# gouldberg/robotics-path-planning

Measured on AMD Instinct MI355X. Metric: RRT* edge expansions/sec + final path cost, 100k-node tree (collision-checked edges evaluated on the device, distinct per iteration; 105000 iterations), higher is better.
Workload: dtype f64

## Files before the change

### robotics-path-planning_amd/csrc/rrt_kernels.hip.h

```cpp
#pragma once
#include <hip/hip_runtime.h>
#include <stdint.h>

#include "rpp_core.h"
#include "rpp_node.h"
#include "rpp_rs.h"

namespace rppk {

constexpr int TPB = 256;
constexpr int NW = TPB / 64;
constexpr int UNROLL = 4;
constexpr int WAVE_STRIDE = 128 * UNROLL;
constexpr int MAX_OBS = 256;
constexpr int NU_MAX = 512;
constexpr int EB = 64;
constexpr int EBD = 32;
constexpr int FCAP = TPB;
constexpr double FILTER_EPS = 7.105427357601002e-15;

struct Result {
  double path_cost;
  int32_t n_nodes;
  int32_t status;
// ... 33 lines not shown
  int32_t *parent, *prev_sib;
  Kid* kid;
  GHead* ghead;
  int32_t *hits, *stack;
  int64_t stride;
  const double *ox, *oy, *othr;
  const double* r2tab;
  double* path_xy;
  int32_t path_cap;
  Result* results;
  int32_t algo, sampler, goal_sample_rate, max_iter, has_play, until_max;
  double rand_min, rand_max, expand_dis, res;
  double play_area[4];
  int32_t trace_inst;
  double *tr_rx, *tr_ry;
  int32_t *tr_near, *tr_nn;
  int32_t* tr_kind;
  float *xf, *yf;
  double f32_m;
  uint32_t* xq;
  double q_lo, q_inv, q_step, q_m;
  const int32_t* inst_map;
  int32_t spec2;
  uint64_t *gent, *gpool;
  int32_t gsh, gn, gcells, gpool_blocks;
  int32_t grid;
  int32_t grid_min;
  int32_t prop_vec, prop_cap;
  int32_t obs_cull;
  int32_t grid_merge;
  int32_t has_elen;
  Node* node;
  double* samp;
};
constexpr int GRID_CAP0 = 16, GRID_CAP1 = 16;

__device__ __forceinline__ uint32_t quant16(const Ctx& c, double px, double py) {
  double qx = __builtin_rint((px - c.q_lo) * c.q_inv), qy = __builtin_rint((py - c.q_lo) * c.q_inv);
  qx = qx < 0.0 ? 0.0 : (qx > 65535.0 ? 65535.0 : qx);
  qy = qy < 0.0 ? 0.0 : (qy > 65535.0 ? 65535.0 : qy);
  return ((uint32_t)qx | ((uint32_t)qy << 16)) ^ 0x80008000u;
}

struct Sh {
  static constexpr int kNU = NU_MAX, kTPB = TPB, kNW = NW;
  rpp::MT rng;
  double ox[MAX_OBS], oy[MAX_OBS], othr[MAX_OBS];
  rpp::Edge edge[EB];
  int32_t ecoll[EB];
  double uval[NU_MAX];
  int32_t uidx[NU_MAX];
  double uex[NU_MAX], uey[NU_MAX], uaux[NU_MAX];
  int32_t usafe[NU_MAX];
  double cval[TPB];
  int32_t cflag[TPB];
  double red_best[NW], red_second[NW];
  int32_t red_idx[NW];
  int32_t wave_cnt[NW];
  int32_t wave_start[NW];
  double rx, ry, nx, ny, ncost, wx, wy, wcost;
  int32_t ni, flag, nu, nvalid, sel, overflow;
  int32_t fa, fb, fover, fcount;
};

__device__ __forceinline__ int roundup_i(int a, int b) { return (a + b - 1) / b * b; }

typedef double v2d __attribute__((ext_vector_type(2)));
__device__ __forceinline__ v2d stream2(const double* p) {
// ... 1239 lines not shown
```

### robotics-path-planning_amd/csrc/rrt_star_v2_grid.inc

```
struct GridS {
  GHead* head;
  uint64_t* ent;
  uint64_t* pool;
  int sh, gn, pool_blocks, pool_next, excl, min_n;
  uint32_t goal_q;
  int ok;
  int merge;
  int bytes, nodes;
};
constexpr int GRID_CAP0 = rppk::GRID_CAP0, GRID_CAP1 = rppk::GRID_CAP1, GRID_CAPT = GRID_CAP0 + GRID_CAP1;
constexpr int GE = 4;
static_assert(GRID_CAPT <= 64, "a cell's entries fit one wave");

__device__ __forceinline__ GHead ld_head(const GHead* p) { return *p; }
__device__ __forceinline__ int grid_cell(const GridS& g, uint32_t q) {
  const uint32_t u = q ^ 0x80008000u;
  return (int)((u >> (16 + g.sh)) * (uint32_t)g.gn + ((u & 0xffffu) >> g.sh));
}
__device__ __forceinline__ uint64_t grid_entry(int node, uint32_t q) { return (uint64_t)(uint32_t)node | ((uint64_t)q << 32); }

__device__ __forceinline__ void grid_build(GridS& g, const uint32_t* __restrict__ xq, const double* x, const double* y,
                                           int n, double gx, double gy, int first_goal) {
  const int lane = threadIdx.x & 63;
  const int cells = g.gn * g.gn;
  for (int i = lane; i < cells; i += 64) {
    g.head[i] = GHead{0, 0};
  }
  g.pool_next = 0;
  g.excl = 0;
  __threadfence();
  const uint64_t lt_mask = (lane == 0) ? 0ull : (~0ull >> (64 - lane));
  for (int i0 = 0; i0 < n; i0 += 64) {
    const int i = i0 + lane;
    bool on = i < n;
    const uint32_t q = on ? xq[i] : 0u;
    if (on && first_goal >= 0 && q == g.goal_q && i != first_goal && x[i] == gx && y[i] == gy) on = false;
    g.excl += __popcll(__ballot(i < n && !on));
    const int cell = grid_cell(g, q);
    const int k = on ? atomicAdd(&g.head[cell].cnt, 1) : 0;
    const uint64_t nb = __ballot(on && k == GRID_CAP0);
    if (on && k == GRID_CAP0) {
// ... 28 lines not shown
        return;
      }
      b = ++g.pool_next;
    }
    if (threadIdx.x == 0) g.pool[(int64_t)(b - 1) * GRID_CAP1 + (k - GRID_CAP0)] = e;
  }
  if (threadIdx.x == 0) g.head[cell] = GHead{k + 1, b};
}

__device__ __forceinline__ void grid_remove(GridS& g, int node, uint32_t q) {
  const int lane = threadIdx.x & 63;
  const int cell = grid_cell(g, q);
  const GHead hd = ld_head(g.head + cell);
  const int k = hd.cnt, b = hd.blk;
  if (k > GRID_CAPT) {
    g.ok = 0;
    return;
  }
  uint64_t* p = lane < GRID_CAP0 ? g.ent + (int64_t)cell * GRID_CAP0 + lane
                                 : (b > 0 ? g.pool + (int64_t)(b - 1) * GRID_CAP1 + (lane - GRID_CAP0) : nullptr);
  const bool mine = lane < k && p != nullptr;
  const uint64_t e = mine ? *p : 0ull;
  const uint64_t m = __ballot(mine && (int)(uint32_t)e == node);
  if (m == 0ull) {
    g.ok = 0;
    return;
  }
  const int j = __ffsll((long long)m) - 1;
  const uint32_t lo = (uint32_t)__shfl((int)(uint32_t)e, k - 1), hi = (uint32_t)__shfl((int)(uint32_t)(e >> 32), k - 1);
  if (lane == j) *p = (uint64_t)lo | ((uint64_t)hi << 32);
  if (lane == 0) g.head[cell].cnt = k - 1;
}

__device__ __forceinline__ int grid_tests(const GridS& g, uint32_t cq, int D, bool ball, uint32_t thr, bool nearest,
                                          const uint32_t (&ev)[GE], const int (&ei)[GE], const uint32_t (&d)[GE],
                                          int32_t* __restrict__ hits, int off, int cap, int32_t* lhit, int32_t* ltmp,
                                          int gz, int& cnt, int& zcnt, uint32_t& best, uint32_t& second, int& grp,
                                          uint32_t& wbest) {
  const int lane = threadIdx.x & 63;
  const uint64_t lt_mask = (lane == 0) ? 0ull : (~0ull >> (64 - lane));
  if (ball) {
    const bool zin = g.excl > 0 && qdist(g.goal_q, cq) <= thr;
    if (zin && gz < 0) return 0;
    int z = zin ? g.excl : 0, H = 0;
    bool hh[GE];
#pragma unroll
    for (int k = 0; k < GE; k++) {
      hh[k] = d[k] <= thr;
      if (gz >= 0) {
        const bool skip = hh[k] && ev[k] == g.goal_q && ei[k] != gz;
        z += __popcll(__ballot(skip));
        hh[k] = hh[k] && !skip;
      }
      const uint64_t m = __ballot(hh[k]);
      if (hh[k]) ltmp[H + __popcll(m & lt_mask)] = ei[k];
      H += __popcll(m);
    }
    lds_barrier();
    for (int h0 = 0; h0 < H; h0 += 64) {
      if (h0 + lane < H) {
        const int me = ltmp[h0 + lane];
        int r = 0;
        for (int j = 0; j < H; j++) r += ltmp[j] < me ? 1 : 0;
        if (r < cap) hits[off + r] = me;
        if (lhit && r < HWF) lhit[r] = me;
      }
    }
    lds_barrier();
    cnt = H;
    zcnt = z;
  }
  if (!nearest) return 1;
  uint32_t b = 0xffffffffu, s = 0xffffffffu;
  int bi = 0x7fffffff;
#pragma unroll
  for (int k = 0; k < GE; k++) {
    if (d[k] < b || (d[k] == b && ei[k] < bi)) {
      s = b;
      b = d[k];
      bi = ei[k];
    } else {
      s = min(s, d[k]);
    }
  }
  uint32_t wb = b;
  int wi = bi;
#pragma unroll
  for (int o = 32; o >= 1; o >>= 1) {
    const uint32_t ob = (uint32_t)__shfl_xor((int)wb, o);
    const int oi = __shfl_xor(wi, o);
    const bool take = ob < wb || (ob == wb && oi < wi);
    wb = take ? ob : wb;
    wi = take ? oi : wi;
  }
  uint32_t ws = bi == wi ? s : b;
#pragma unroll
  for (int o = 32; o >= 1; o >>= 1) ws = min(ws, (uint32_t)__shfl_xor((int)ws, o));
  if (g.excl > 0) ws = min(ws, qdist(g.goal_q, cq));
  wbest = wb;
  if (wb < QSAT && (double)D > __builtin_sqrt((double)wb) + 4.0) {
    best = wb;
    second = min(ws, (uint32_t)(D * D));
    grp = wi & ~3;
    return 1;
  }
  return 2;
}

__device__ __forceinline__ bool grid_window(const GridS& g, uint32_t cq, int rw, int& x0, int& y0, int& nwx, int& nc, int& D) {
  const int ux = (int)((cq ^ 0x80008000u) & 0xffffu), uy = (int)((cq ^ 0x80008000u) >> 16);
  x0 = max(ux - rw, 0) >> g.sh;
  y0 = max(uy - rw, 0) >> g.sh;
  const int x1 = min(ux + rw, 65535) >> g.sh, y1 = min(uy + rw, 65535) >> g.sh;
  nwx = x1 - x0 + 1;
  nc = nwx * (y1 - y0 + 1);
  if (nc > 64) return false;
  D = 32767;
  if (x0 > 0) D = min(D, ux - (x0 << g.sh) + 1);
  if (x1 < g.gn - 1) D = min(D, ((x1 + 1) << g.sh) - ux);
  if (y0 > 0) D = min(D, uy - (y0 << g.sh) + 1);
  if (y1 < g.gn - 1) D = min(D, ((y1 + 1) << g.sh) - uy);
  return true;
}

__device__ __forceinline__ int grid_grow(uint32_t wb, int rw) { return wb < QSAT ? (int)__builtin_sqrt((double)wb) + 6 : 3 * rw + 1; }

__device__ __forceinline__ bool grid_centre(const GridS& g, uint32_t cq, int rw, bool ball, uint32_t thr, bool nearest,
                                            int32_t* __restrict__ hits, int off, int cap, int32_t* lhit, int32_t* ltmp,
                                            int gz, int& cnt, int& zcnt, uint32_t& best, uint32_t& second, int& grp,
                                            int& bytes, int& nodes, int first_attempt = 0) {
  const int lane = threadIdx.x & 63;
  for (int attempt = first_attempt; attempt < 3; attempt++) {
    int x0, y0, nwx, nc, D;
    if (!grid_window(g, cq, rw, x0, y0, nwx, nc, D)) return false;
    int cell = 0, cn = 0, cb = 0;
    if (lane < nc) {
      cell = (y0 + lane / nwx) * g.gn + x0 + lane % nwx;
      const GHead hd = ld_head(g.head + cell);
      cn = hd.cnt;
      cb = hd.blk;
    }
    if (__ballot(cn > GRID_CAPT) != 0ull) return false;
    int inc = cn;
#pragma unroll
    for (int o = 1; o < 64; o <<= 1) {
      const int t = __shfl_up(inc, o);
      if (lane >= o) inc += t;
    }
    const int tot = __shfl(inc, 63);
    bytes += 8 * nc + 8 * tot;
    nodes += tot;
    if (tot > 64 * GE) return false;
    const int pre = inc - cn;
    const uint64_t* ptr[GE];
#pragma unroll
    for (int k = 0; k < GE; k++) ptr[k] = nullptr;
    for (uint64_t nz = __ballot(cn > 0); nz != 0ull; nz &= nz - 1) {
      const int j = __ffsll((long long)nz) - 1;
      const int pj = __builtin_amdgcn_readlane(pre, j), cj = __builtin_amdgcn_readlane(cn, j);
      const int ej = __builtin_amdgcn_readlane(cell, j), bj = __builtin_amdgcn_readlane(cb, j);
#pragma unroll
      for (int k = 0; k < GE; k++) {
        const int r = lane + 64 * k - pj;
        if (r >= 0 && r < cj)
          ptr[k] = r < GRID_CAP0 ? g.ent + (int64_t)ej * GRID_CAP0 + r : g.pool + (int64_t)(bj - 1) * GRID_CAP1 + (r - GRID_CAP0);
      }
    }
    uint32_t ev[GE], d[GE];
    int ei[GE];
#pragma unroll
    for (int k = 0; k < GE; k++) {
      const uint64_t e = ptr[k] ? *ptr[k] : 0ull;
      ei[k] = ptr[k] ? (int)(uint32_t)e : 0x7fffffff;
      ev[k] = (uint32_t)(e >> 32);
      d[k] = ptr[k] ? qdist(ev[k], cq) : 0xffffffffu;
    }
    uint32_t wb = 0xffffffffu;
    const int r = grid_tests(g, cq, D, ball && attempt == 0, thr, nearest, ev, ei, d, hits, off, cap, lhit, ltmp, gz, cnt,
                             zcnt, best, second, grp, wb);
    if (r != 2) return r == 1;
    rw = grid_grow(wb, rw);
    ball = false;
  }
  return false;
}

struct GCen {
  uint32_t cq, thr;
  int rw;
  bool on, ball, nearest;
  int off, cap, gz;
  int32_t* lhit;
  int cnt, zcnt, grp;
  uint32_t best, second;
};

template <int NC>
__device__ __forceinline__ int grid_merged(const GridS& g, GCen (&ce)[NC], int32_t* __restrict__ hits, int32_t* ltmp,
                                           int& bytes, int& nodes, uint32_t& grow) {
  const int lane = threadIdx.x & 63;
  int D[NC], npairs = 0;
  int cid = -1, cell = 0, cn = 0, cb = 0;
#pragma unroll
  for (int c = 0; c < NC; c++) {
    D[c] = 0;
    if (!ce[c].on) continue;
    int x0, y0, nwx, nc;
    if (!grid_window(g, ce[c].cq, ce[c].rw, x0, y0, nwx, nc, D[c])) return -1;
    const int l = lane - npairs;
    if (l >= 0 && l < nc) {
      cid = c;
      cell = (y0 + l / nwx) * g.gn + x0 + l % nwx;
    }
    npairs += nc;
  }
  if (npairs > 64) return -1;
  if (cid >= 0) {
    const GHead hd = ld_head(g.head + cell);
    cn = hd.cnt;
    cb = hd.blk;
  }
  if (__ballot(cn > GRID_CAPT) != 0ull) return 0;
  int inc = cn;
#pragma unroll
  for (int o = 1; o < 64; o <<= 1) {
// ... 19 lines not shown
    sc[k] = -1;
    if (slot < tot) {
      int j = 0;
#pragma unroll
      for (int st = 32; st >= 1; st >>= 1)
        if (ltmp[j + st - 1] <= slot) j += st;
      const int r = slot - (j > 0 ? ltmp[j - 1] : 0);
      const int ej = ltmp[64 + j], bj = ltmp[128 + j];
      sc[k] = ltmp[192 + j];
      ptr[k] = r < GRID_CAP0 ? g.ent + (int64_t)ej * GRID_CAP0 + r : g.pool + (int64_t)(bj - 1) * GRID_CAP1 + (r - GRID_CAP0);
    }
  }
#pragma unroll
  for (int k = 0; k < GE; k++) {
    const uint64_t e = ptr[k] ? *ptr[k] : 0ull;
    ei[k] = (int)(uint32_t)e;
    ev[k] = (uint32_t)(e >> 32);
  }
  lds_barrier();
  grow = 0u;
#pragma unroll
  for (int c = 0; c < NC; c++) {
    if (!ce[c].on) continue;
    uint32_t d[GE];
    int eic[GE];
#pragma unroll
    for (int k = 0; k < GE; k++) {
      const bool mine = sc[k] == c;
      eic[k] = mine ? ei[k] : 0x7fffffff;
      d[k] = mine ? qdist(ev[k], ce[c].cq) : 0xffffffffu;
    }
    uint32_t wb = 0xffffffffu;
    const int r = grid_tests(g, ce[c].cq, D[c], ce[c].ball, ce[c].thr, ce[c].nearest, ev, eic, d, hits, ce[c].off, ce[c].cap,
                             ce[c].lhit, ltmp, ce[c].gz, ce[c].cnt, ce[c].zcnt, ce[c].best, ce[c].second, ce[c].grp, wb);
    if (r == 0) return 0;
    if (r == 2) {
      grow |= 1u << c;
      ce[c].best = wb;
    }
  }
  return 1;
}

template <bool NEAR, bool NEAREST, int KS>
__device__ __forceinline__ bool grid_pass(GridS& g, int rwn, uint32_t qq, uint32_t thr, uint32_t sq,
                                          int32_t* __restrict__ hits, Sh2& sh, int& ggrp, double& gbest, double& gsecond,
                                          int gz, int* zskip, SpecQ* sp, int& total) {
  int32_t* lhit = reinterpret_cast<int32_t*>(sh.u.hit);
  int32_t* ltmp = lhit + HWF;
  static_assert(sizeof(sh.u) >= sizeof(int32_t) * (HWF + 64 * GE), "LDS scratch of a grid pass");
  int bytes = 0, nodes = 0;
  uint32_t b, s;
  int gr, zc = 0, cnt = 0;
  if (g.merge) {
    GCen ce[KS + 2];
    ce[0].on = NEAR;
    ce[0].cq = qq; ce[0].thr = thr; ce[0].rw = (int)__builtin_sqrt((double)thr) + 1;
    ce[0].ball = true; ce[0].nearest = false;
    ce[0].off = 0; ce[0].cap = 0x7fffffff; ce[0].gz = gz; ce[0].lhit = lhit;
    ce[0].cnt = 0; ce[0].zcnt = 0; ce[0].grp = 0x7ffffffc; ce[0].best = ce[0].second = 0xffffffffu;
#pragma unroll
    for (int j = 0; j <= KS; j++) {
      GCen& e = ce[1 + j];
      const int jo = j < KS ? j : 0;
      e.cq = j == 0 ? sq : sp[j > 0 ? j - 1 : 0].sq;
      e.nearest = j == 0 ? NEAREST : sp[j > 0 ? j - 1 : 0].thr != 0u;
      e.thr = j < KS ? sp[jo].thr : 0u;
      e.ball = e.thr != 0u;
      e.on = e.nearest || e.ball;
      e.rw = max(e.ball ? (int)__builtin_sqrt((double)e.thr) + 1 : 0, e.nearest ? rwn : 0);
      e.off = KS > 0 ? sp[jo].off : 0;
      e.cap = KS > 0 ? sp[jo].cap : 0;
      e.gz = -1;
      e.lhit = nullptr;
      e.cnt = 0; e.zcnt = 0; e.grp = 0x7ffffffc; e.best = e.second = 0xffffffffu;
    }
    uint32_t grow = 0u;
    const int r = grid_merged<KS + 2>(g, ce, hits, ltmp, bytes, nodes, grow);
    if (r == 0) return false;
    if (r == 1) {
#pragma unroll
      for (int j = 0; j <= KS; j++) {
        GCen& e = ce[1 + j];
        if (grow >> (1 + j) & 1u) {
          int bc, bz;
          const uint32_t wb = e.best;
          e.best = e.second = 0xffffffffu;
          if (!grid_centre(g, e.cq, grid_grow(wb, e.rw), false, 0u, true, hits, 0, 0, nullptr, ltmp, -1, bc, bz, e.best,
                           e.second, e.grp, bytes, nodes, 1))
            return false;
        }
        if (j == 0) {
          if (NEAREST) {
            gbest = (double)e.best;
            gsecond = (double)e.second;
            ggrp = e.grp;
          }
        } else {
          sp[j - 1].best = (double)e.best;
          sp[j - 1].second = (double)e.second;
          sp[j - 1].grp = e.grp;
        }
        if (j < KS) sp[j < KS ? j : 0].cnt = e.cnt;
      }
      if (NEAR && threadIdx.x == 0) {
        sh.wave_cnt[0] = ce[0].cnt;
        sh.wave_start[0] = 0;
        sh.fa = ce[0].zcnt;
      }
      lds_barrier();
      if (NEAR && zskip) *zskip = gz >= 0 ? ce[0].zcnt : 0;
      total = NEAR ? ce[0].cnt : 0;
      g.bytes = bytes;
      g.nodes = nodes;
      return true;
    }
  }
  if (NEAR) {
    const int rw = (int)__builtin_sqrt((double)thr) + 1;
    if (!grid_centre(g, qq, rw, true, thr, false, hits, 0, 0x7fffffff, lhit, ltmp, gz, cnt, zc, b, s, gr, bytes, nodes))
      return false;
  }
#pragma unroll
  for (int j = 0; j <= KS; j++) {
    const uint32_t cq = j == 0 ? sq : sp[j > 0 ? j - 1 : 0].sq;
    const bool nq = j == 0 ? NEAREST : sp[j > 0 ? j - 1 : 0].thr != 0u;
    const uint32_t bthr = j < KS ? sp[j < KS ? j : 0].thr : 0u;
    uint32_t bb = 0xffffffffu, bs = 0xffffffffu;
    int bg = 0x7ffffffc, bc = 0, bz = 0;
    if (nq || bthr != 0u) {
      const int rw = max(bthr != 0u ? (int)__builtin_sqrt((double)bthr) + 1 : 0, nq ? rwn : 0);
      const int jo = j < KS ? j : 0;
      if (!grid_centre(g, cq, rw, bthr != 0u, bthr, nq, hits, KS > 0 ? sp[jo].off : 0, KS > 0 ? sp[jo].cap : 0, nullptr,
                       ltmp, -1, bc, bz, bb, bs, bg, bytes, nodes))
        return false;
    }
    if (j == 0) {
      if (NEAREST) {
        gbest = (double)bb;
        gsecond = (double)bs;
        ggrp = bg;
      }
    } else {
      sp[j - 1].best = (double)bb;
      sp[j - 1].second = (double)bs;
      sp[j - 1].grp = bg;
    }
    if (j < KS) sp[j < KS ? j : 0].cnt = bc;
  }
  if (NEAR && threadIdx.x == 0) {
    sh.wave_cnt[0] = cnt;
    sh.wave_start[0] = 0;
    sh.fa = zc;
  }
  lds_barrier();
  if (NEAR && zskip) *zskip = gz >= 0 ? zc : 0;
  total = NEAR ? cnt : 0;
  g.bytes = bytes;
  g.nodes = nodes;
  return true;
}

template <bool NEAR, bool NEAREST, int KS = 0>
__device__ __forceinline__ int scan2g(GridS& g, int rwn, const uint32_t* __restrict__ xq, int n, uint32_t qq, uint32_t thr,
                                      uint32_t sq, int32_t* __restrict__ hits, Sh2& sh, int& ggrp, double& gbest,
                                      double& gsecond, uint32_t gq = 0u, int gz = -1, int* zskip = nullptr,
                                      SpecQ* sp = nullptr) {
  if constexpr (NW == 1) {
    if (g.ok && n >= g.min_n) {
      int total = 0;
      if (grid_pass<NEAR, NEAREST, KS>(g, rwn, qq, thr, sq, hits, sh, ggrp, gbest, gsecond, gz, zskip, sp, total))
        return total;
    }
  }
  g.bytes = 4 * n;
  g.nodes = n;
  return scan2q<NEAR, NEAREST, KS>(xq, n, qq, thr, sq, hits, sh, ggrp, gbest, gsecond, gq, gz, zskip, sp);
}
```

### robotics-path-planning_amd/csrc/rrt_star_v2_kernel.inc

```
#define ST_ADD(k, v) do { if (threadIdx.x == 0) sh.stat[k] += (long long)(v); } while (0)
enum { S_ITER, S_EU, S_ER, S_NH, S_NU, S_RW, S_PR, S_SN, S_AB, S_AB2, S_EX, S_NUMAX, S_FB, S_QA, S_RIDE };
__device__ __forceinline__ uint32_t ball_thr_grid(double r2, double qm, double qinv) {
  const double rr = __builtin_sqrt(r2) + qm;
  const double thr_gd = rr * rr * qinv * qinv * (1.0 + 1e-6) + 1.0;
  return thr_gd < 4.0e9 ? (uint32_t)thr_gd : 4000000000u;
}
__device__ __forceinline__ bool on_goal(int first_goal, double gx, double gy, double sx, double sy) {
  return first_goal >= 0 && sx == gx && sy == gy;
}
__device__ __forceinline__ void nearest_on_goal(int first_goal, double gx, double gy, int& ni, double& nx, double& ny,
                                                double& best, double& second) {
  ni = first_goal;
  nx = gx;
  ny = gy;
  best = 0.0;
  second = rpp::dinf();
}
template <bool SECOND, class At, class Keep, class Dist>
__device__ __forceinline__ void hit_argmin(int k, At at, Keep keep, Dist dist, Sh2& sh, double& gbest, int& gidx,
                                           double& gsecond, double& gx, double& gy) {
  double best = rpp::dinf(), second = rpp::dinf(), bx = 0.0, by = 0.0;
  int bidx = 0x7fffffff;
  for (int h = threadIdx.x; h < k; h += TPB) {
    int idx;
// ... 54 lines not shown
  int goal_dups = I->goal_dups;

  const int om = uni_i(I->obs_m);
  {
    const int ob = uni_i(I->obs_base);
    for (int i = tid; i < om; i += TPB) {
      sh.ox[i] = c.ox[ob + i];
      sh.oy[i] = c.oy[ob + i];
      sh.othr[i] = c.othr[ob + i];
    }
    if (tid == 0) {
      sh.overflow = 0;
      sh.om = om;
    }
  }
  lds_barrier();
  int n = __builtin_amdgcn_readfirstlane(I->n), it = __builtin_amdgcn_readfirstlane(I->it);
  const double gx = I->goal[0], gy = I->goal[1];
  const v2d* S = reinterpret_cast<const v2d*>(c.samp) + (int64_t)inst * c.max_iter;
  GridS gs = {};
  gs.ok = 0;
  if constexpr (NW == 1) {
    if (c.grid) {
      const int64_t gi = (int64_t)inst;
      gs.head = c.ghead + gi * c.gcells;
      gs.ent = c.gent + gi * c.gcells * GRID_CAP0;
      gs.pool = c.gpool + gi * c.gpool_blocks * GRID_CAP1;
      gs.sh = c.gsh;
      gs.gn = c.gn;
      gs.pool_blocks = c.gpool_blocks;
      gs.min_n = c.grid_min;
      gs.merge = c.grid_merge;
      gs.goal_q = goal_q;
      gs.ok = 1;
      grid_build(gs, xq, x, y, n, gx, gy, first_goal);
    }
  }
  {
    const double* cost = c.cost + off;
    const Kid* kid = c.kid + off;
    const int32_t* parent = c.parent + off;
    const int32_t* prev_sib = c.prev_sib + off;
    for (int i = tid; i < n; i += TPB) {
      Node r;
      r.k = kid[i];
      r.cost = cost[i];
      r.parent = parent[i];
      r.prev_sib = prev_sib[i];
      r.x = x[i];
      r.y = y[i];
      r.xq = xq[i];
      r.pad[0] = r.pad[1] = r.pad[2] = 0u;
      nd[i] = r;
    }
    asm volatile("s_waitcnt vmcnt(0)" ::: "memory");
    lds_barrier();
  }
  if (tid == 0)
    for (int k = 0; k < 15; k++) sh.stat[k] = 0;
  int have_nearest = 0, ni = 0;
  double gbest = 0.0, gsecond = 0.0, nqx = 0.0, nqy = 0.0;
  int stop = 0;
  constexpr int SPEC_CAPS = 2048 / (KSM > 0 ? KSM : 1);
  const int spec_base = (int)c.stride - 2048;
  const int KS_RUN = NW == 1 ? (c.spec2 < KSM ? c.spec2 : KSM) : 0;
  const bool SPEC_ON = KS_RUN > 0;
// ... 11 lines not shown
    double axv[4], ayv[4];
#pragma unroll
    for (int j = 0; j < 4; j++) {
      axv[j] = sh.ax[j];
      ayv[j] = sh.ay[j];
    }
    o_bq = 0xffffffffu;
    if (grpd < 0.0) return 0;
    if (on_goal(first_goal, gx, gy, s2x, s2y)) {
      nearest_on_goal(first_goal, gx, gy, ni, nqx, nqy, gbest, gsecond);
      return 1;
    }
    double dl = rpp::dinf(), lx = 0.0, ly = 0.0;
    int li = 0;
#pragma unroll
    for (int j = 0; j < 4; j++) {
      if (j < na) {
        const double dxl = axv[j] - s2x, dyl = ayv[j] - s2y;
        const double d1 = __builtin_sqrt(dxl * dxl + dyl * dyl);
        if (d1 < dl) {
          dl = d1;
          li = B_n + j;
          lx = axv[j];
          ly = ayv[j];
        }
      }
    }
    const double db = __builtin_sqrt(nb), ds = __builtin_sqrt(nsec);
    const uint32_t bq = (uint32_t)bqd;
    const int grp = (int)grpd;
    gbest = 1.0;
    gsecond = rpp::dinf();
    if (margin_fold(c, qm, dl, li, lx, ly, db, ds, bq, grp, B_n, rppk::quant16(c, s2x, s2y),
                    [&](double& hx, double& hy) { hx = x[grp + (tid & 3)]; hy = y[grp + (tid & 3)]; },
                    ni, nqx, nqy))
      return 1;
    o_bq = bq;
    return bq < QSAT ? 2 : 0;
  };
  PH_DECL

  for (int step = 0; step < iters && it < c.max_iter && !stop; step++, it++) {
    ST_ADD(S_ITER, 1);
    double rx, ry;
    sload_sample(S, it, rx, ry);
    PH(0);
    ST_ADD(S_AB2, 16 * (int64_t)n);
    const double r2 = c.r2tab[n + 1];
    const double r2b = SPEC_ON ? c.r2tab[n + 2] : 0.0;
    if (!have_nearest) {
      bool done = false;
      if (on_goal(first_goal, gx, gy, rx, ry)) {
        nearest_on_goal(first_goal, gx, gy, ni, nqx, nqy, gbest, gsecond);
        done = true;
      } else {
        const uint32_t sq = rppk::quant16(c, rx, ry);
        uint32_t bq = q_amb_bq;
        bool bound = q_amb != 0;
        if (!bound) {
          int grp;
          double fb, fs;
          scan2g<false, true>(gs, (int)(__builtin_sqrt(r2) * qinv) + 1, xq, n, 0u, 0u, sq, hits, sh, grp, fb, fs);
          ST_ADD(S_SN, gs.nodes);
          ST_ADD(S_AB, gs.bytes + 64);
          if (fb < (double)QSAT) {
            if ((__builtin_sqrt(fs) - __builtin_sqrt(fb)) > 2.0 * qm_grid) {
              const int gl = grp + (tid & 3);
// ... 131 lines not shown
    PH(2);
    const double nx = sh.nx, ny = sh.ny;
    const int inplay = sh.flag;
    if (inplay && ext_exact) {
      ST_ADD(S_EU, 1);
      ST_ADD(S_ER, 1);
      for (int k = tid, mk = uni_i(sh.om); k < mk; k += TPB)
        if (rpp::edge_hits_obstacle(sh.e0, sh.ox[k], sh.oy[k], sh.othr[k])) sh.ecoll0 = 1;
    }
    lds_barrier();
    const int accepted = inplay && !sh.ecoll0;
    int nnear = -1;
    PH(3);

    if (accepted) {
      bool use_spec = false;
      int spec_k0 = 0, spec_off0 = 0;
      if (SPEC_ON && ns > 0) {
        const double* R = sh.set[shead];
        const double cx0 = R[0], cy0 = R[1], k0 = R[4], o0 = R[5];
        use_spec = uni_i(k0 >= 0.0 && nx == cx0 && ny == cy0) != 0;
        spec_k0 = uni_i((int)k0);
        spec_off0 = uni_i((int)o0);
      }
      bool did_spec = false;
      const int do_pf = !use_spec && (step + 1 < iters) && (it + 1 < c.max_iter);
      int kraw;
      int pf_ni = 0;
      double pf_best = 0.0, pf_second = 0.0, pf_x = 0.0, pf_y = 0.0;
      int zskip = 0;
      const int zgate = (first_goal >= 0 && goal_dups > 0) ? first_goal : -1;
      uint32_t pf_sq = 0u, pf_bq = 0u;
      int pf_grp = -1, pf_n = 0;
      bool pf_goal = false;
      double p1x = 0.0, p1y = 0.0;
      int64_t pass_b = 0, pass_n = n;
      if (use_spec) {
        int k2 = spec_k0;
        const int off0 = spec_off0;
        const uint32_t cq = rppk::quant16(c, nx, ny);
        double axv[KA], ayv[KA];
#pragma unroll
        for (int j = 0; j < KA; j++) {
          axv[j] = sh.ax[j];
          ayv[j] = sh.ay[j];
        }
#pragma unroll
        for (int j = 0; j < KA; j++) {
          if (uni_i(j < na && qdist(rppk::quant16(c, axv[j], ayv[j]), cq) <= B_thr)) {
            if (tid == 0) hits[off0 + k2] = B_n + j;
            k2++;
          }
        }
        asm volatile("s_waitcnt vmcnt(0)" ::: "memory");
        int32_t* lhit = reinterpret_cast<int32_t*>(sh.u.hit);
        for (int h = tid; h < k2 && h < HWF; h += TPB) lhit[h] = hits[off0 + h];
        if (tid == 0) {
          sh.wave_cnt[0] = k2;
          sh.wave_start[0] = off0;
        }
        lds_barrier();
        kraw = k2;
        ST_ADD(S_RIDE, 1);
        ST_ADD(S_AB, 16 * (int64_t)kraw + 16);
      } else {
        ns = 0;
        na = 0;
        const uint32_t thr_gi = ball_thr_grid(r2, qm, qinv);
        const int rw_gi = (int)__builtin_sqrt((double)thr_gi) + 1;
        if (do_pf) {
          sload_sample(S, it + 1, p1x, p1y);
          pf_goal = on_goal(first_goal, gx, gy, p1x, p1y);
        }
        if (do_pf && !pf_goal) {
          pf_sq = rppk::quant16(c, p1x, p1y);
          int kmax = 0;
          if (SPEC_ON && n >= 256) {
            kmax = iters - step - 2 < c.max_iter - it - 2 ? iters - step - 2 : c.max_iter - it - 2;
            kmax = kmax < 0 ? 0 : (kmax > KS_RUN ? KS_RUN : kmax);
          }
          kmax = uni_i(kmax);
          if constexpr (NW == 1 && KSM > 0) {
            uint32_t thr2 = 0u;
            if (kmax > 0) {
              thr2 = ball_thr_grid(r2b, qm, qinv);
              if (uni_i(qdist(goal_q, pf_sq) <= thr2)) kmax = 0;
            }
            if (kmax > 0) {
              double qxv[KA], qyv[KA];
// ... 15 lines not shown
                const bool on = j < ks;
                const double cxj = j == 0 ? p1x : qxv[j > 0 ? j - 1 : 0], cyj = j == 0 ? p1y : qyv[j > 0 ? j - 1 : 0];
                sp[j].qq = on ? rppk::quant16(c, cxj, cyj) : pf_sq;
                sp[j].thr = on ? thr2 : 0u;
                sp[j].sq = rppk::quant16(c, on ? qxv[j] : p1x, on ? qyv[j] : p1y);
                sp[j].off = spec_base + j * SPEC_CAPS;
                sp[j].cap = SPEC_CAPS;
                if (tid == 0) {
                  double* R = sh.set[j];
                  R[0] = cxj;
                  R[1] = cyj;
                  R[5] = (double)sp[j].off;
                }
              }
              kraw = scan2g<true, true, KSM>(gs, rw_gi, xq, n, rppk::quant16(c, nx, ny), thr_gi, pf_sq, hits, sh, pf_ni,
                                             pf_best, pf_second, goal_q, zgate, &zskip, sp);
              pass_b = gs.bytes;
              pass_n = gs.nodes;
              did_spec = true;
              B_n = n;
              B_thr = uni_u(thr2);
              ns = ks;
              shead = 0;
              na = 0;
              if (tid == 0) {
                const double qs2 = c.q_step * c.q_step;
#pragma unroll
                for (int j = 0; j < KA; j++) {
                  const bool on = j < ks;
                  double* R = sh.set[j];
                  R[2] = sp[j].best * qs2;
                  R[3] = sp[j].second * qs2;
                  R[4] = (on && sp[j].cnt + j + 1 <= SPEC_CAPS) ? (double)sp[j].cnt : -1.0;
                  R[6] = on ? (double)sp[j].grp : -1.0;
                  R[7] = sp[j].best;
                }
              }
            }
          }
          if (!did_spec) {
            kraw = scan2g<true, true>(gs, rw_gi, xq, n, rppk::quant16(c, nx, ny), thr_gi, pf_sq, hits, sh, pf_ni, pf_best,
                                      pf_second, goal_q, zgate, &zskip);
            pass_b = gs.bytes;
            pass_n = gs.nodes;
          }
          if (zskip > goal_dups) {
            kraw = scan2g<true, true>(gs, rw_gi, xq, n, rppk::quant16(c, nx, ny), thr_gi, pf_sq, hits, sh, pf_ni, pf_best,
                                      pf_second);
            zskip = 0;
            ST_ADD(S_AB, gs.bytes);
          }
          pf_bq = (uint32_t)pf_best;
          pf_grp = pf_ni;
          pf_n = n;
          pf_x = x[pf_grp + (tid & 3)];
          pf_y = y[pf_grp + (tid & 3)];
          pf_best *= c.q_step * c.q_step;
          pf_second *= c.q_step * c.q_step;
        } else {
          int d0;
          double d1, d2;
          kraw = scan2g<true, false>(gs, rw_gi, xq, n, rppk::quant16(c, nx, ny), thr_gi, 0u, hits, sh, d0, d1, d2, goal_q,
                                     zgate, &zskip);
          pass_b = gs.bytes;
          pass_n = gs.nodes;
          if (zskip > goal_dups) {
            kraw = scan2g<true, false>(gs, rw_gi, xq, n, rppk::quant16(c, nx, ny), thr_gi, 0u, hits, sh, d0, d1, d2);
            zskip = 0;
            ST_ADD(S_AB, gs.bytes);
          }
        }
        ST_ADD(S_AB, pass_b + 16 * (int64_t)kraw + 16);
      }
      ST_ADD(S_SN, pass_n);
      ST_ADD(S_AB2, 16 * (int64_t)n);
      auto fold_new_node = [&](double ax, double ay, int aidx, int& o_ni, double& o_x, double& o_y) -> int {
        if (pf_goal) {
          nearest_on_goal(first_goal, gx, gy, o_ni, o_x, o_y, pf_best, pf_second);
          return 1;
        }
        const double dxl = ax - p1x, dyl = ay - p1y;
        const double dl = __builtin_sqrt(dxl * dxl + dyl * dyl);
        const double db = __builtin_sqrt(pf_best), ds = __builtin_sqrt(pf_second);
        return margin_fold(c, qm, dl, aidx, ax, ay, db, ds, pf_bq, pf_grp, pf_n, pf_sq,
                           [&](double& hx, double& hy) { hx = pf_x; hy = pf_y; }, o_ni, o_x, o_y);
      };
      PH(4);
      int pend_p, pend_fc;
      double pend_cost;
// ... 195 lines not shown
      } else {
        if (tid == 0) {
          x[n] = nx;
          y[n] = ny;
          xq[n] = rppk::quant16(c, nx, ny);
          const double el = rpp::py_hypot(nx - nqx, ny - nqy);
          nd[n].k.elen = el;
          nd[n].cost = nd[ni].cost + el;
          nd[n].k.first_child = -1;
          nd[n].x = nx;
          nd[n].y = ny;
          nd[n].xq = rppk::quant16(c, nx, ny);
          link_child_rec(nd, n, ni);
          sh.moved = 0;
        }
        if (gs.ok) {
          if (first_goal >= 0 && nx == gx && ny == gy)
            gs.excl++;
          else
            grid_insert(gs, n, rppk::quant16(c, nx, ny));
        }
        n++;
        lds_barrier();
      }
      const int moved = uni_i(sh.moved);
      if (moved & 2) first_goal = -2;
      if ((moved & 2) && gs.excl > 0) gs.ok = 0;
      if (wx == gx && wy == gy) {
        if (first_goal == -1) {
          first_goal = n - 1;
          goal_dups = 0;
        } else if (first_goal >= 0) {
          goal_dups++;
        }
      }
      if (do_pf && !moved) {
        have_nearest = fold_new_node(wx, wy, n - 1, pf_ni, pf_x, pf_y);
        if (!have_nearest && pf_bq < QSAT) {
          q_amb = 1;
          q_amb_bq = pf_bq;
        }
        pf_best = pf_goal ? 0.0 : 1.0;
        pf_second = rpp::dinf();
      }
      if (tid == 0 && inst == c.trace_inst) {
        c.tr_rx[it] = rx;
        c.tr_ry[it] = ry;
        c.tr_near[it] = ni;
        c.tr_nn[it] = nnear;
        c.tr_kind[it] = have ? 2 : 1;
      }
      ni = pf_ni;
      gbest = pf_best;
      gsecond = pf_second;
      nqx = pf_x;
      nqy = pf_y;
      if (SPEC_ON) {
        if (moved) {
          ns = 0;
          na = 0;
        } else if ((use_spec || did_spec) && na < 4) {
          if (tid == 0) {
            sh.ax[na] = wx;
            sh.ay[na] = wy;
          }
          na++;
// ... 86 lines not shown
```

### robotics-path-planning_amd/csrc/rrt_star_v2_shapes.inc

```
using rppk::Ctx;
using rppk::Inst;
using rppk::Kid;
using rppk::Node;
using rppk::GHead;
using rppk::FILTER_EPS;
using rppk::v2d;
using rppk::stream2;
using rppk::roundup_i;

constexpr int TPB = RRT2_TPB;
constexpr int NW = TPB / 64;
#ifndef RRT2_UNROLL
#define RRT2_UNROLL 4
#endif
constexpr int UNROLL = RRT2_UNROLL;
constexpr int WAVE_STRIDE = 128 * UNROLL;
constexpr int MAX_OBS = RRT2_MAXOBS;
constexpr int NU = RRT2_NU;
constexpr int EBD = RRT2_EBD;
constexpr int HW = RRT2_HW;
constexpr int FCAP = RRT2_FCAP;
constexpr int WPS = RRT2_WPS;

struct Hit {
  double x, y;
  int32_t idx, pad;
};
struct Front {
  double c, x, y;
  int32_t idx, fc;
};
struct WalkEnt {
  double cp;
  int32_t node, pad;
};

struct Sh2 {
  double ox[MAX_OBS], oy[MAX_OBS], othr[MAX_OBS];
  union {
    Hit hit[NW * HW];
    rpp::Edge edge[2 * EBD];
    WalkEnt walk[2 * FCAP * (int)(sizeof(Front) / sizeof(WalkEnt))];
  } u;
  rpp::Edge e0;
  double cval[TPB];
  int32_t cflag[TPB];
  int32_t uidx[NU], ufc[NU], uflag[NU];
  double ux[NU], uy[NU], ucur[NU], uval[NU], uhyp[NU], uex[NU], uey[NU];
  double red_best[NW], red_second[NW], red_x[NW], red_y[NW];
  int32_t red_idx[NW], wave_cnt[NW], wave_start[NW];
  double nx, ny;
  int32_t flag, nu, nvalid, overflow, ecoll0;
  int32_t fa, fb, fover, fcount;
  int32_t n_rw, n_pr, moved, last_fc;
  int32_t om;
  long long stat[15];
  double ax[4], ay[4];
  double set[4][8];
};

__device__ __forceinline__ void lds_barrier() { __syncthreads(); }
__device__ __forceinline__ int uni_i(int v) { return __builtin_amdgcn_readfirstlane(v); }
__device__ __forceinline__ uint32_t uni_u(uint32_t v) { return (uint32_t)__builtin_amdgcn_readfirstlane((int)v); }
__device__ __forceinline__ double uni_d(double v) {
  const uint64_t b = rpp::d2b(v);
  const uint32_t lo = uni_u((uint32_t)b), hi = uni_u((uint32_t)(b >> 32));
  return rpp::b2d(((uint64_t)hi << 32) | lo);
}

__device__ __forceinline__ void block_argmin_xy(double best, int bidx, double second, double bx, double by, Sh2& sh,
                                                double& gbest, int& gidx, double& gsecond, double& gx, double& gy) {
  const int lane = threadIdx.x & 63, w = threadIdx.x >> 6;
  double b = best;
  int bi = bidx;
#pragma unroll
  for (int o = 32; o >= 1; o >>= 1) {
    double ob = __shfl_xor(b, o);
    int oi = __shfl_xor(bi, o);
    bool take = (ob < b) || (ob == b && oi < bi);
    b = take ? ob : b;
    bi = take ? oi : bi;
  }
  double s = (bidx == bi) ? second : best;
#pragma unroll
  for (int o = 32; o >= 1; o >>= 1) {
    double os = __shfl_xor(s, o);
    s = os < s ? os : s;
  }
  const uint64_t own = __ballot(bidx == bi);
  const int owner = own ? (__ffsll((long long)own) - 1) : 0;
  const double wx = __shfl(bx, owner), wy = __shfl(by, owner);
// ... 59 lines not shown
```

### robotics-path-planning_amd/csrc/rrtx_api.hip

```cpp
#include <algorithm>
#include <chrono>
#include <cstdio>
#include <functional>
#include <mutex>
#include <new>
#include <set>
#include <vector>

#include "rrtx_host.h"
#include "rrt_kernels.hip.h"
#include "rrt_star_v2.hip.h"
#include "rrt_samples.hip.h"
#include "rrt_informed.hip.h"
#include "rrt_dubins.hip.h"
#include "rrt_rs.hip.h"
#include "rrt_bitstar.hip.h"
#include "rrt_bitstar_wave.hip.h"
#include "path_smooth.hip.h"
#include "rrt_lqr.hip.h"
#include "rrt_track.hip.h"
#include "course_gather.hip.h"
#include "goal_query.hip.h"
#include "goal_track.hip.h"
#include "steer_batch.hip.h"
// ... 198 lines not shown
  const V2Shape& s = v2_shape(tpb);
  return timed_launch(h, false, [&] { hipLaunchKernelGGL(s.kernel, dim3(nblk), dim3(s.tpb), 0, h->stream, c, h->v2_chunk_iters); });
}
static int launch_sample_stream(rrtx_handle* h, const Ctx& c, int nblk) {
  float ms = 0.f;
  int rc = h->timed(&ms, [&] { hipLaunchKernelGGL(rppss::rrt_sample_stream_kernel, dim3(nblk), dim3(64), 0, h->stream, c); });
  if (rc) return rc;
  h->run.kms += ms;
  return RRTX_OK;
}
static int launch_rrt_star_v2(rrtx_handle* h, const Ctx& c, int nblk, int tpb) {
  for (int64_t done_it = 0; done_it < c.max_iter; done_it += h->v2_chunk_iters) {
    int rc = launch_rrt_star_v2_once(h, c, nblk, tpb);
    if (rc) return rc;
  }
  return RRTX_OK;
}

static void rrt_star_knobs(Ctx& c) {
  c.spec2 = 8;
  if (const char* e = getenv("RRTX_SPEC2")) c.spec2 = atoi(e) > 0 ? atoi(e) : 0;
  c.grid = c.ghead != nullptr;
  if (const char* e = getenv("RRTX_GRID")) c.grid = c.grid && atoi(e) != 0;
  c.grid_min = 4096;
  if (const char* e = getenv("RRTX_GRID_MIN")) c.grid_min = atoi(e) > 0 ? atoi(e) : 0;
  c.prop_vec = 8;
  if (const char* e = getenv("RRTX_PROP_VEC")) c.prop_vec = atoi(e);
  c.prop_cap = 1 << 30;
  if (const char* e = getenv("RRTX_PROP_CAP")) c.prop_cap = atoi(e) > 0 ? atoi(e) : 0;
  c.obs_cull = 1;
  if (const char* e = getenv("RRTX_OBS_CULL")) c.obs_cull = atoi(e) != 0;
  c.grid_merge = 1;
  if (const char* e = getenv("RRTX_GRID_MERGE")) c.grid_merge = atoi(e) != 0;
}

static int estimate_near_capacity(const rrtx_params& p) {
  const double n = (double)p.max_iter + 1.0;
  const double side = fabs(p.rand_max - p.rand_min);
  const double area = side * side > 1e-12 ? side * side : 1e-12;
  double a = p.connect_circle_dist * p.connect_circle_dist * log(n > 2.0 ? n : 2.0), b = n * p.expand_dis * p.expand_dis;
  const double lam = M_PI * (a < b ? a : b) / area;
  const double cap = lam + 6.0 * sqrt(lam) + 8.0;
  return cap > 1e6 ? 1000000 : (int)cap;
}

static void rccl_release(rrtx_handle* h);
static void handle_register(const rrtx_handle* h);
static void handle_unregister(const rrtx_handle* h);

extern "C" {

int rrtx_abi_version(void) { return RRTX_ABI_VERSION; }

int rrtx_device_count(void) {
  int n = 0;
  if (hipGetDeviceCount(&n) != hipSuccess) return 0;
  return n;
}

const char* rrtx_last_error(rrtx_handle* h) { return h ? h->err.c_str() : "null handle"; }

void rrtx_destroy(rrtx_handle* h) {
  if (!h) return;
  handle_unregister(h);
  hipSetDevice(h->device);
  rccl_release(h);
// ... 1397 lines not shown
```

Baseline: 1.976 billion.

## Keep speculative near-lists and group coordinates in LDS instead of global memory

When the grid search runs with a single wave, the speculative neighbour lists for up to three look-ahead samples are written to shared-memory buffers instead of the global hits array, provided they fit a capacity limit. The kernel then copies the list into the capture buffer straight from LDS, which removes the global write/read round trip and the vmcnt wait. Speculative group coordinates are also cached in LDS so that the margin fold reads them from there rather than from global x/y. The cost is extra LDS use and more branching, plus a new environment knob to set the capacity.

```diff
diff --git a/robotics-path-planning_amd/csrc/rrt_kernels.hip.h b/robotics-path-planning_amd/csrc/rrt_kernels.hip.h
--- a/robotics-path-planning_amd/csrc/rrt_kernels.hip.h
+++ b/robotics-path-planning_amd/csrc/rrt_kernels.hip.h
@@ -89,8 +89,10 @@
   int32_t has_elen;
   Node* node;
   double* samp;
+  int32_t spec_lds;
 };
 constexpr int GRID_CAP0 = 16, GRID_CAP1 = 16;
+constexpr int SPEC_LDS_MAX = 64;
 
 __device__ __forceinline__ uint32_t quant16(const Ctx& c, double px, double py) {
   double qx = __builtin_rint((px - c.q_lo) * c.q_inv), qy = __builtin_rint((py - c.q_lo) * c.q_inv);
diff --git a/robotics-path-planning_amd/csrc/rrt_star_v2_grid.inc b/robotics-path-planning_amd/csrc/rrt_star_v2_grid.inc
--- a/robotics-path-planning_amd/csrc/rrt_star_v2_grid.inc
+++ b/robotics-path-planning_amd/csrc/rrt_star_v2_grid.inc
@@ -7,6 +7,7 @@
   int ok;
   int merge;
   int bytes, nodes;
+  int spec_lds;
 };
 constexpr int GRID_CAP0 = rppk::GRID_CAP0, GRID_CAP1 = rppk::GRID_CAP1, GRID_CAPT = GRID_CAP0 + GRID_CAP1;
 constexpr int GE = 4;
@@ -101,11 +102,13 @@
   if (lane == 0) g.head[cell].cnt = k - 1;
 }
 
+__device__ __forceinline__ bool spec_fits(int lcap, int H) { return lcap >= 0 && H <= lcap; }
+
 __device__ __forceinline__ int grid_tests(const GridS& g, uint32_t cq, int D, bool ball, uint32_t thr, bool nearest,
                                           const uint32_t (&ev)[GE], const int (&ei)[GE], const uint32_t (&d)[GE],
-                                          int32_t* __restrict__ hits, int off, int cap, int32_t* lhit, int32_t* ltmp,
-                                          int gz, int& cnt, int& zcnt, uint32_t& best, uint32_t& second, int& grp,
-                                          uint32_t& wbest) {
+                                          int32_t* __restrict__ hits, int off, int cap, int32_t* lhit, int lcap,
+                                          int32_t* ltmp, int gz, int& cnt, int& zcnt, uint32_t& best, uint32_t& second,
+                                          int& grp, uint32_t& wbest) {
   const int lane = threadIdx.x & 63;
   const uint64_t lt_mask = (lane == 0) ? 0ull : (~0ull >> (64 - lane));
   if (ball) {
@@ -126,13 +129,15 @@
       H += __popcll(m);
     }
     lds_barrier();
+    const bool in_lds = spec_fits(lcap, H);
+    const int ltop = lcap == -1 ? HWF : (in_lds ? H : 0);
     for (int h0 = 0; h0 < H; h0 += 64) {
       if (h0 + lane < H) {
         const int me = ltmp[h0 + lane];
         int r = 0;
         for (int j = 0; j < H; j++) r += ltmp[j] < me ? 1 : 0;
-        if (r < cap) hits[off + r] = me;
-        if (lhit && r < HWF) lhit[r] = me;
+        if (!in_lds && r < cap) hits[off + r] = me;
+        if (lhit && r < ltop) lhit[r] = me;
       }
     }
     lds_barrier();
@@ -195,9 +200,9 @@
 __device__ __forceinline__ int grid_grow(uint32_t wb, int rw) { return wb < QSAT ? (int)__builtin_sqrt((double)wb) + 6 : 3 * rw + 1; }
 
 __device__ __forceinline__ bool grid_centre(const GridS& g, uint32_t cq, int rw, bool ball, uint32_t thr, bool nearest,
-                                            int32_t* __restrict__ hits, int off, int cap, int32_t* lhit, int32_t* ltmp,
-                                            int gz, int& cnt, int& zcnt, uint32_t& best, uint32_t& second, int& grp,
-                                            int& bytes, int& nodes, int first_attempt = 0) {
+                                            int32_t* __restrict__ hits, int off, int cap, int32_t* lhit, int lcap,
+                                            int32_t* ltmp, int gz, int& cnt, int& zcnt, uint32_t& best, uint32_t& second,
+                                            int& grp, int& bytes, int& nodes, int first_attempt = 0) {
   const int lane = threadIdx.x & 63;
   for (int attempt = first_attempt; attempt < 3; attempt++) {
     int x0, y0, nwx, nc, D;
@@ -245,14 +250,17 @@
       d[k] = ptr[k] ? qdist(ev[k], cq) : 0xffffffffu;
     }
     uint32_t wb = 0xffffffffu;
-    const int r = grid_tests(g, cq, D, ball && attempt == 0, thr, nearest, ev, ei, d, hits, off, cap, lhit, ltmp, gz, cnt,
-                             zcnt, best, second, grp, wb);
+    const int r = grid_tests(g, cq, D, ball && attempt == 0, thr, nearest, ev, ei, d, hits, off, cap, lhit, lcap, ltmp, gz,
+                             cnt, zcnt, best, second, grp, wb);
     if (r != 2) return r == 1;
     rw = grid_grow(wb, rw);
     ball = false;
   }
   return false;
 }
+
+__device__ __forceinline__ int32_t* spec_list(Sh2& sh, int j) { return sh.slist[NW == 1 && j < 3 ? j : 0]; }
+__device__ __forceinline__ int spec_room(const GridS& g, int j) { return g.spec_lds >= j + 1 ? g.spec_lds - (j + 1) : -2; }
 
 struct GCen {
   uint32_t cq, thr;
@@ -260,6 +268,7 @@
   bool on, ball, nearest;
   int off, cap, gz;
   int32_t* lhit;
+  int lcap;
   int cnt, zcnt, grp;
   uint32_t best, second;
 };
@@ -345,7 +354,8 @@
     }
     uint32_t wb = 0xffffffffu;
     const int r = grid_tests(g, ce[c].cq, D[c], ce[c].ball, ce[c].thr, ce[c].nearest, ev, eic, d, hits, ce[c].off, ce[c].cap,
-                             ce[c].lhit, ltmp, ce[c].gz, ce[c].cnt, ce[c].zcnt, ce[c].best, ce[c].second, ce[c].grp, wb);
+                             ce[c].lhit, ce[c].lcap, ltmp, ce[c].gz, ce[c].cnt, ce[c].zcnt, ce[c].best, ce[c].second,
+                             ce[c].grp, wb);
     if (r == 0) return 0;
     if (r == 2) {
       grow |= 1u << c;
@@ -370,7 +380,7 @@
     ce[0].on = NEAR;
     ce[0].cq = qq; ce[0].thr = thr; ce[0].rw = (int)__builtin_sqrt((double)thr) + 1;
     ce[0].ball = true; ce[0].nearest = false;
-    ce[0].off = 0; ce[0].cap = 0x7fffffff; ce[0].gz = gz; ce[0].lhit = lhit;
+    ce[0].off = 0; ce[0].cap = 0x7fffffff; ce[0].gz = gz; ce[0].lhit = lhit; ce[0].lcap = -1;
     ce[0].cnt = 0; ce[0].zcnt = 0; ce[0].grp = 0x7ffffffc; ce[0].best = ce[0].second = 0xffffffffu;
 #pragma unroll
     for (int j = 0; j <= KS; j++) {
@@ -385,7 +395,8 @@
       e.off = KS > 0 ? sp[jo].off : 0;
       e.cap = KS > 0 ? sp[jo].cap : 0;
       e.gz = -1;
-      e.lhit = nullptr;
+      e.lhit = spec_list(sh, jo);
+      e.lcap = spec_room(g, jo);
       e.cnt = 0; e.zcnt = 0; e.grp = 0x7ffffffc; e.best = e.second = 0xffffffffu;
     }
     uint32_t grow = 0u;
@@ -399,7 +410,7 @@
           int bc, bz;
           const uint32_t wb = e.best;
           e.best = e.second = 0xffffffffu;
-          if (!grid_centre(g, e.cq, grid_grow(wb, e.rw), false, 0u, true, hits, 0, 0, nullptr, ltmp, -1, bc, bz, e.best,
+          if (!grid_centre(g, e.cq, grid_grow(wb, e.rw), false, 0u, true, hits, 0, 0, nullptr, -1, ltmp, -1, bc, bz, e.best,
                            e.second, e.grp, bytes, nodes, 1))
             return false;
         }
@@ -431,7 +442,7 @@
   }
   if (NEAR) {
     const int rw = (int)__builtin_sqrt((double)thr) + 1;
-    if (!grid_centre(g, qq, rw, true, thr, false, hits, 0, 0x7fffffff, lhit, ltmp, gz, cnt, zc, b, s, gr, bytes, nodes))
+    if (!grid_centre(g, qq, rw, true, thr, false, hits, 0, 0x7fffffff, lhit, -1, ltmp, gz, cnt, zc, b, s, gr, bytes, nodes))
       return false;
   }
 #pragma unroll
@@ -444,8 +455,8 @@
     if (nq || bthr != 0u) {
       const int rw = max(bthr != 0u ? (int)__builtin_sqrt((double)bthr) + 1 : 0, nq ? rwn : 0);
       const int jo = j < KS ? j : 0;
-      if (!grid_centre(g, cq, rw, bthr != 0u, bthr, nq, hits, KS > 0 ? sp[jo].off : 0, KS > 0 ? sp[jo].cap : 0, nullptr,
-                       ltmp, -1, bc, bz, bb, bs, bg, bytes, nodes))
+      if (!grid_centre(g, cq, rw, bthr != 0u, bthr, nq, hits, KS > 0 ? sp[jo].off : 0, KS > 0 ? sp[jo].cap : 0,
+                       spec_list(sh, jo), spec_room(g, jo), ltmp, -1, bc, bz, bb, bs, bg, bytes, nodes))
         return false;
     }
     if (j == 0) {
@@ -482,8 +493,12 @@
   if constexpr (NW == 1) {
     if (g.ok && n >= g.min_n) {
       int total = 0;
-      if (grid_pass<NEAR, NEAREST, KS>(g, rwn, qq, thr, sq, hits, sh, ggrp, gbest, gsecond, gz, zskip, sp, total))
+      if (grid_pass<NEAR, NEAREST, KS>(g, rwn, qq, thr, sq, hits, sh, ggrp, gbest, gsecond, gz, zskip, sp, total)) {
+#pragma unroll
+        for (int j = 0; j < KS; j++)
+          if (spec_fits(spec_room(g, j), sp[j].cnt)) sp[j].off = -1;
         return total;
+      }
     }
   }
   g.bytes = 4 * n;
diff --git a/robotics-path-planning_amd/csrc/rrt_star_v2_kernel.inc b/robotics-path-planning_amd/csrc/rrt_star_v2_kernel.inc
--- a/robotics-path-planning_amd/csrc/rrt_star_v2_kernel.inc
+++ b/robotics-path-planning_amd/csrc/rrt_star_v2_kernel.inc
@@ -110,6 +110,7 @@
       gs.min_n = c.grid_min;
       gs.merge = c.grid_merge;
       gs.goal_q = goal_q;
+      gs.spec_lds = KSM == 3 ? (c.spec_lds < SPEC_L ? (c.spec_lds > 0 ? c.spec_lds : 0) : SPEC_L) : 0;
       gs.ok = 1;
       grid_build(gs, xq, x, y, n, gx, gy, first_goal);
     }
@@ -187,7 +188,7 @@
     gbest = 1.0;
     gsecond = rpp::dinf();
     if (margin_fold(c, qm, dl, li, lx, ly, db, ds, bq, grp, B_n, rppk::quant16(c, s2x, s2y),
-                    [&](double& hx, double& hy) { hx = x[grp + (tid & 3)]; hy = y[grp + (tid & 3)]; },
+                    [&](double& hx, double& hy) { hx = sh.gx[4 * (shead & 3) + (tid & 3)]; hy = sh.gy[4 * (shead & 3) + (tid & 3)]; },
                     ni, nqx, nqy))
       return 1;
     o_bq = bq;
@@ -385,6 +386,7 @@
       const int zgate = (first_goal >= 0 && goal_dups > 0) ? first_goal : -1;
       uint32_t pf_sq = 0u, pf_bq = 0u;
       int pf_grp = -1, pf_n = 0;
+      int pf_gl = -1;
       bool pf_goal = false;
       double p1x = 0.0, p1y = 0.0;
       int64_t pass_b = 0, pass_n = n;
@@ -398,16 +400,28 @@
           axv[j] = sh.ax[j];
           ayv[j] = sh.ay[j];
         }
+        int32_t* lhit = reinterpret_cast<int32_t*>(sh.u.hit);
+        static_assert(SPEC_L <= HWF, "a list from LDS fits the capture");
+        const bool in_lds = NW == 1 && off0 < 0;
 #pragma unroll
         for (int j = 0; j < KA; j++) {
           if (uni_i(j < na && qdist(rppk::quant16(c, axv[j], ayv[j]), cq) <= B_thr)) {
-            if (tid == 0) hits[off0 + k2] = B_n + j;
+            if (tid == 0) {
+              if (in_lds)
+                lhit[k2] = B_n + j;
+              else
+                hits[off0 + k2] = B_n + j;
+            }
             k2++;
           }
         }
-        asm volatile("s_waitcnt vmcnt(0)" ::: "memory");
-        int32_t* lhit = reinterpret_cast<int32_t*>(sh.u.hit);
-        for (int h = tid; h < k2 && h < HWF; h += TPB) lhit[h] = hits[off0 + h];
+        if (in_lds) {
+          const int32_t* sl = sh.slist[NW == 1 ? shead & 3 : 0];
+          for (int h = tid; h < spec_k0; h += TPB) lhit[h] = sl[h];
+        } else {
+          asm volatile("s_waitcnt vmcnt(0)" ::: "memory");
+          for (int h = tid; h < k2 && h < HWF; h += TPB) lhit[h] = hits[off0 + h];
+        }
         if (tid == 0) {
           sh.wave_cnt[0] = k2;
           sh.wave_start[0] = off0;
@@ -489,10 +503,14 @@
                   R[2] = sp[j].best * qs2;
                   R[3] = sp[j].second * qs2;
                   R[4] = (on && sp[j].cnt + j + 1 <= SPEC_CAPS) ? (double)sp[j].cnt : -1.0;
+                  R[5] = (double)sp[j].off;
                   R[6] = on ? (double)sp[j].grp : -1.0;
                   R[7] = sp[j].best;
                 }
               }
+#pragma unroll
+              for (int j = 0; j < KA; j++)
+                if ((tid >> 2) == j + 1) pf_gl = (j < ks && sp[j].grp >= 0 && sp[j].grp < n) ? sp[j].grp : 0;
             }
           }
           if (!did_spec) {
@@ -510,8 +528,14 @@
           pf_bq = (uint32_t)pf_best;
           pf_grp = pf_ni;
           pf_n = n;
-          pf_x = x[pf_grp + (tid & 3)];
-          pf_y = y[pf_grp + (tid & 3)];
+          if (did_spec) {
+            const v2d gxy = *reinterpret_cast<const v2d*>(&nd[(pf_gl >= 0 ? pf_gl : pf_grp) + (tid & 3)].x);
+            pf_x = gxy.x;
+            pf_y = gxy.y;
+          } else {
+            pf_x = x[pf_grp + (tid & 3)];
+            pf_y = y[pf_grp + (tid & 3)];
+          }
           pf_best *= c.q_step * c.q_step;
           pf_second *= c.q_step * c.q_step;
         } else {
@@ -773,6 +797,12 @@
           goal_dups = 0;
         } else if (first_goal >= 0) {
           goal_dups++;
+        }
+      }
+      if constexpr (NW == 1) {
+        if (did_spec && tid >= 4 && tid < 16) {
+          sh.gx[tid - 4] = pf_x;
+          sh.gy[tid - 4] = pf_y;
         }
       }
       if (do_pf && !moved) {
diff --git a/robotics-path-planning_amd/csrc/rrt_star_v2_shapes.inc b/robotics-path-planning_amd/csrc/rrt_star_v2_shapes.inc
--- a/robotics-path-planning_amd/csrc/rrt_star_v2_shapes.inc
+++ b/robotics-path-planning_amd/csrc/rrt_star_v2_shapes.inc
@@ -21,6 +21,7 @@
 constexpr int HW = RRT2_HW;
 constexpr int FCAP = RRT2_FCAP;
 constexpr int WPS = RRT2_WPS;
+constexpr int SPEC_L = rppk::SPEC_LDS_MAX;
 
 struct Hit {
   double x, y;
@@ -57,6 +58,8 @@
   long long stat[15];
   double ax[4], ay[4];
   double set[4][8];
+  int32_t slist[NW == 1 ? 3 : 1][NW == 1 ? SPEC_L : 1];
+  double gx[NW == 1 ? 12 : 1], gy[NW == 1 ? 12 : 1];
 };
 
 __device__ __forceinline__ void lds_barrier() { __syncthreads(); }
diff --git a/robotics-path-planning_amd/csrc/rrtx_api.hip b/robotics-path-planning_amd/csrc/rrtx_api.hip
--- a/robotics-path-planning_amd/csrc/rrtx_api.hip
+++ b/robotics-path-planning_amd/csrc/rrtx_api.hip
@@ -254,6 +254,11 @@
   if (const char* e = getenv("RRTX_OBS_CULL")) c.obs_cull = atoi(e) != 0;
   c.grid_merge = 1;
   if (const char* e = getenv("RRTX_GRID_MERGE")) c.grid_merge = atoi(e) != 0;
+  c.spec_lds = rppk::SPEC_LDS_MAX;
+  if (const char* e = getenv("RRTX_SPEC_LDS")) {
+    const int v = atoi(e);
+    c.spec_lds = v < 0 ? 0 : (v > rppk::SPEC_LDS_MAX ? rppk::SPEC_LDS_MAX : v);
+  }
 }
 
 static int estimate_near_capacity(const rrtx_params& p) {
```

After: 2.011 billion, median of 6. 1.02x the previous value.
